# sylvainma/Summarizer

Hardware: NVIDIA B200
Metric: VASNet/DSN frames/sec fwd+bwd and knapsack-eval videos/sec at 1/2/4/8 B200 (higher is better)
Workload: dtype bf16 (tcgen05 operands, fp32 accumulate/softmax/LayerNorm); i32/u8 eval

## Files before the change

include/summarizer_b200.h:

```cpp
#ifndef SUMMARIZER_B200_H
#define SUMMARIZER_B200_H

#include <stdint.h>

#ifdef __cplusplus
extern "C" {
#endif

#define SMZ_OK 0
#define SMZ_ERR_ARG (-1)
#define SMZ_ERR_CUDA (-2)
#define SMZ_ERR_UNSUPPORTED (-3)
#define SMZ_ERR_NCCL (-4)
#define SMZ_ERR_DEVICE (-5)

#define SMZ_METHOD_KNAPSACK 0
#define SMZ_METHOD_RANK 1

#define SMZ_STATUS_VALUE_RANGE 1
#define SMZ_STATUS_INTERVALS 2
#define SMZ_STATUS_WEIGHT_RANGE 4

#define SMZ_FSCORE_CHUNK 2048

// ... 49 lines not shown

int smz_upsample(const smz_video_desc *desc, int n_videos, int max_n_frames, const float *scores,
                 const int32_t *picks, float *frame_scores, int32_t *status, void *stream);

#define SMZ_METRIC_SPEARMAN 0
#define SMZ_METRIC_KENDALL 1
typedef struct smz_corr_desc {
    int64_t m_off, u_off, u_ld, rank_off;
    int32_t n_frames, n_users, row0, reserved;
} smz_corr_desc;
int smz_rank_correlation(const smz_corr_desc *desc, int n_videos, int max_n_frames, int max_n_users,
                         const float *machine, const float *user, int metric, float *rank_ws, double *corr,
                         double *corr_avg, void *stream);

#define SMZ_OPTIM_MAX_TENSORS 64
typedef struct smz_optim_tensor {
    float *param, *grad, *exp_avg, *exp_avg_sq, *step;
    int64_t n;
} smz_optim_tensor;
int smz_grad_sqnorm_workspace_floats(const smz_optim_tensor *tensors, int n_tensors, int64_t *floats);
int smz_grad_sqnorm(const smz_optim_tensor *tensors, int n_tensors, float *sqnorm, float *ws, int64_t ws_floats, void *stream);
int smz_clip_grads(const smz_optim_tensor *tensors, int n_tensors, const float *sqnorm, float max_norm, void *stream);
int smz_adam_step(const smz_optim_tensor *tensors, int n_tensors, double lr, double beta1, double beta2, double eps,
                  double weight_decay, void *stream);
int smz_mse_loss(const float *scores, const float *target, int64_t n, float *loss, float *dscores, void *stream);

#define SMZ_GEMM_OUT_F32 1
#define SMZ_GEMM_RELU 2
#define SMZ_GEMM_RES_F32 4
#define SMZ_GEMM_BIAS_M 8
#define SMZ_GEMM_OUT_F16 2048
#define SMZ_GEMM_A_F16 4096
#define SMZ_GEMM_B_F16 8192
int smz_gemm_bf16_tn(const void *A, int64_t lda, const void *B, int64_t ldb, void *C, int64_t ldc, int M, int N,
                     int K, float alpha, const float *bias, const void *residual, int64_t ldr, int flags,
                     void *stream);
int smz_cvt_bf16_multi(const float *const *src, void *const *dst, const int64_t *n, int count, void *stream);
int smz_gemm_bf16(int a_mn, int b_mn, const void *A, int64_t lda, const void *B, int64_t ldb, void *C, int64_t ldc,
                  int M, int N, int K, float alpha, const float *bias, const void *residual, int64_t ldr, int flags,
                  void *stream);
int smz_gemm_bf16_split(int a_mn, int b_mn, const void *A, const void *A_lo, int64_t lda, const void *B,
                        const void *B_lo, int64_t ldb, void *C, void *C_lo, int64_t ldc, int M, int N, int K, float alpha,
                        const float *bias, const void *residual, int64_t ldr, int flags, void *stream);
int smz_split_bf16_multi(const float *const *src, void *const *hi, void *const *lo, const int64_t *n, int count,
                         void *stream);

#define SMZ_VASNET_STATUS_LOGIT_RANGE 1
#define SMZ_VASNET_STATUS_F16_RANGE 2
typedef struct smz_vasnet_params {
    const void *wqk, *wv, *wo, *w1;
    const float *b1, *w2, *b2, *ln_g, *ln_b;
    float scale, eps;
    int32_t aperture, ignore_self;
    const float *head_gw, *head_c;
    const void *w1g;
    const float *ln_c, *b1f;
    const void *wgv, *wgv16;
    int32_t *status;
    const void *wqk_lo, *wv_lo, *wo_lo, *w1_lo;
} smz_vasnet_params;
#define SMZ_VASNET_SPLIT 4

int smz_dropout_keep_masks(uint64_t *state, uint8_t *out, int64_t n, void *stream);
int smz_vasnet_workspace_bytes(const int32_t *h_cu_seqlens, int n_videos, int training, int x_is_bf16,
                               int64_t *bytes);
void smz_vasnet_set_exact_softmax(int on);
// ... 110 lines not shown
```

summarizer_b200/csrc/smz_gemm.cu:

```cuda
#include "smz_gemm.cuh"
#include "smz_tc.cuh"

#include <cudaTypedefs.h>
#include <stdlib.h>

namespace {

using namespace smztc;
using smz::GemmEpilogue;
using smz::GemmProblem;

constexpr int BM = 128;
constexpr int BN = smz::GEMM_BN, BK = smz::GEMM_BK;
constexpr int A_STAGE = BM * BK * 2;
constexpr int EPI_WARPS = 8;
constexpr int NUM_THREADS = 64 + 32 * EPI_WARPS;
constexpr int TMEM_COLS = 2 * BN;
constexpr int BAR_BYTES = 256;
constexpr int STG_BYTES = EPI_WARPS * 32 * 33 * 4;
static_assert(TMEM_COLS == 512, "TMEM allocation must be a power of two <= 512 columns");
template <bool PAIR> struct Cfg {
    static constexpr int STAGES = PAIR ? 5 : 3;
    static constexpr int B_ROWS = PAIR ? BN / 2 : BN;
    static constexpr int B_STAGE = B_ROWS * BK * 2;
    static constexpr int TILE_M = PAIR ? 2 * BM : BM;
    static constexpr int SMEM_BYTES = STAGES * (A_STAGE + B_STAGE) + BAR_BYTES + STG_BYTES + 1024;
};

struct Params {
    const GemmProblem *probs;
    GemmProblem single;
    int n_probs, total_tiles;
    GemmEpilogue epi;
};

struct Cursor {
    int p = -1;
    GemmProblem cur;
    __device__ __forceinline__ void seek(const Params &P, int tile) {
        if (P.probs == nullptr) { cur = P.single; return; }
        int q = p < 0 ? 0 : p;
        while (q + 1 < P.n_probs && tile >= __ldg(&P.probs[q + 1].tile0)) ++q;
        if (q != p) { p = q; cur = P.probs[q]; }
    }
};

__device__ __forceinline__ float4 ld_f4(const float *p) { return *reinterpret_cast<const float4 *>(p); }

enum { EPI_PLAIN = 0, EPI_HEAD = 1, EPI_EXP = 2, EPI_SPLIT = 3 };

template <bool A_MN, bool B_MN, bool PAIR, int EPI_T>
__global__ void __launch_bounds__(NUM_THREADS, 1)
gemm_kernel(const __grid_constant__ CUtensorMap tmA, const __grid_constant__ CUtensorMap tmB,
            const __grid_constant__ CUtensorMap tmA_lo, const __grid_constant__ CUtensorMap tmB_lo, const Params P) {
    constexpr bool SPLIT_OUT = EPI_T == EPI_SPLIT;
    constexpr int EPI = SPLIT_OUT ? (int)EPI_PLAIN : EPI_T;
    const int pass_a = P.epi.a_lo != 0 ? 1 : -1;
    const int pass_b = P.epi.b_lo != 0 ? (P.epi.a_lo != 0 ? 2 : 1) : -1;
    const int npass = 1 + (P.epi.a_lo != 0 ? 1 : 0) + (P.epi.b_lo != 0 ? 1 : 0);
    constexpr int STAGES = Cfg<PAIR>::STAGES, B_STAGE = Cfg<PAIR>::B_STAGE, B_ROWS = Cfg<PAIR>::B_ROWS;
    constexpr int TILE_M = Cfg<PAIR>::TILE_M;
    extern __shared__ uint8_t smem_raw[];
    uint8_t *smem = smem_raw + ((1024u - (smem_u32(smem_raw) & 1023u)) & 1023u);
    uint8_t *sA = smem;
    uint8_t *sB = smem + STAGES * A_STAGE;
    uint64_t *full = reinterpret_cast<uint64_t *>(smem + STAGES * (A_STAGE + B_STAGE));
    uint64_t *empty = full + STAGES;
    uint64_t *tfull = empty + STAGES;
    uint64_t *tempty = tfull + 2;
    uint32_t *tmem_slot = reinterpret_cast<uint32_t *>(tempty + 2);
    float *stg_all = reinterpret_cast<float *>(smem + STAGES * (A_STAGE + B_STAGE) + BAR_BYTES);

    smz::pdl_trigger();
    if (P.epi.gate != nullptr) {
        smz::pdl_wait();
        if (__ldg(P.epi.gate) == 0) return;
    }
    const int warp = __shfl_sync(0xffffffffu, threadIdx.x >> 5, 0), lane = threadIdx.x & 31;
    const int rank = PAIR ? (int)cluster_ctarank() : 0;
    const int first_tile = PAIR ? (int)(blockIdx.x >> 1) : (int)blockIdx.x;
    const int tile_step = PAIR ? (int)(gridDim.x >> 1) : (int)gridDim.x;
    if (PAIR) cluster_sync_all();
    if (warp == 0 && lane == 0) {
        tma_prefetch_desc(&tmA);
        tma_prefetch_desc(&tmB);
        if (npass > 1) { tma_prefetch_desc(&tmA_lo); tma_prefetch_desc(&tmB_lo); }
        for (int i = 0; i < STAGES; i++) { mbar_init(&full[i], PAIR ? 2 : 1); mbar_init(&empty[i], 1); }
        for (int i = 0; i < 2; i++) { mbar_init(&tfull[i], 1); mbar_init(&tempty[i], (PAIR ? 2 : 1) * 32 * EPI_WARPS); }
        fence_mbar_init();
    }
    if (warp == 1) { if (PAIR) tmem_alloc_pair<TMEM_COLS>(tmem_slot); else tmem_alloc<TMEM_COLS>(tmem_slot); }
    tc_fence_before();
    if (PAIR) cluster_sync_all(); else __syncthreads();
    tc_fence_after();
// ... 21 lines not shown
                        else if (rank == 0) mbar_arrive_expect_tx(&full[stage], 2 * (A_STAGE + B_STAGE));
                        else mbar_arrive_remote(&full[stage], 0);
                        if (A_MN) {
#pragma unroll
                            for (int j = 0; j < BM / 64; j++)
                                tma_load<PAIR>(sA + stage * A_STAGE + j * 8192, mapA, &full[stage], a_mn + 64 * j, a_k + kb * BK);
                        } else {
                            tma_load<PAIR>(sA + stage * A_STAGE, mapA, &full[stage], a_k + kb * BK, a_mn);
                        }
                        if (B_MN) {
#pragma unroll
                            for (int j = 0; j < B_ROWS / 64; j++)
                                tma_load<PAIR>(sB + stage * B_STAGE + j * 8192, mapB, &full[stage], b_mn + 64 * j, b_k + kb * BK);
                        } else {
                            tma_load<PAIR>(sB + stage * B_STAGE, mapB, &full[stage], b_k + kb * BK, b_mn);
                        }
                    }
                    __syncwarp();
                    if (++stage == STAGES) { stage = 0; phase ^= 1u; }
                }
            }
        }
    } else if (warp == 1) {
        if (rank == 0) {
            Cursor c;
            const uint32_t idesc = (make_idesc_bf16(TILE_M, BN) | (A_MN ? (1u << 15) : 0u) | (B_MN ? (1u << 16) : 0u))
                                   & ~(((P.epi.flags & smz::GEMM_A_F16) ? (1u << 7) : 0u) | ((P.epi.flags & smz::GEMM_B_F16) ? (1u << 10) : 0u));
            const uint32_t a_base = smem_u32(sA), b_base = smem_u32(sB);
            int stage = 0; uint32_t phase = 0;
            int it = 0;
            for (int tile = first_tile; tile < P.total_tiles; tile += tile_step, ++it) {
                c.seek(P, tile);
                const int nkb = ((c.cur.K + BK - 1) / BK) * npass;
                const int as = it & 1;
                mbar_wait(&tempty[as], (((uint32_t)it >> 1) & 1u) ^ 1u);
                tc_fence_after();
                const uint32_t d_tmem = tmem_base + (uint32_t)(as * BN);
                for (int kb = 0; kb < nkb; kb++) {
                    mbar_wait(&full[stage], phase);
                    tc_fence_after();
                    const uint32_t a_addr = a_base + stage * A_STAGE, b_addr = b_base + stage * B_STAGE;
                    const uint64_t adesc = A_MN ? make_mnmajor_sw128_desc(a_addr) : make_kmajor_sw128_desc(a_addr);
                    const uint64_t bdesc = B_MN ? make_mnmajor_sw128_desc(b_addr) : make_kmajor_sw128_desc(b_addr);
                    if (elect_one()) {
#pragma unroll
                        for (int k = 0; k < BK / 16; k++)
                            umma_bf16<PAIR>(d_tmem, adesc + (A_MN ? 128 : 2) * k, bdesc + (B_MN ? 128 : 2) * k, idesc,
                                            (uint32_t)((kb | k) != 0));
                        umma_commit<PAIR>(&empty[stage]);
                    }
                    __syncwarp();
                    if (++stage == STAGES) { stage = 0; phase ^= 1u; }
                }
                if (elect_one()) umma_commit<PAIR>(&tfull[as]);
                __syncwarp();
            }
        }
    } else {
        Cursor c;
        const int q = warp & 3;
        const int half = (warp - 2) >> 2;
        float *stg = stg_all + (warp - 2) * (32 * 33);
        const int row = q * 32 + lane;
        const float alpha = P.epi.alpha;
        const int flags = P.epi.flags;
        int it = 0;
        for (int tile = first_tile; tile < P.total_tiles; tile += tile_step, ++it) {
            c.seek(P, tile);
            const GemmProblem &g = c.cur;
            const int lt = tile - g.tile0;
            const int mt = lt / g.tiles_n, nt = lt - mt * g.tiles_n;
            const int as = it & 1;
            const int m = mt * TILE_M + rank * BM + row;
            const bool row_ok = m < g.M;
            const float bias_m = (P.epi.bias != nullptr && (flags & smz::GEMM_BIAS_M) && !(flags & (smz::GEMM_SCALE_M | smz::GEMM_SCALE_STATS)) && row_ok) ? __ldg(P.epi.bias + m) : 0.f;
            const bool out_f32 = flags & smz::GEMM_OUT_F32;
            const bool res_f32 = flags & smz::GEMM_RES_F32;
            const bool c_vec = ((g.c_off | (int64_t)g.ldc) & 7) == 0 && (reinterpret_cast<uintptr_t>(P.epi.C) & 15) == 0;
            const int64_t res_off = (flags & smz::GEMM_RES_AT_C) ? g.c_off : g.r_off;
            const int res_ld = (flags & smz::GEMM_RES_AT_C) ? g.ldc : g.ldr;
            const bool r_vec = ((res_off | (int64_t)res_ld) & 7) == 0 && (reinterpret_cast<uintptr_t>(P.epi.residual) & 15) == 0;
            const char *res_row = P.epi.residual == nullptr ? nullptr
                : reinterpret_cast<const char *>(P.epi.residual) + (res_off + (int64_t)m * res_ld) * (res_f32 ? 4 : 2);
            auto res_vec_ok = [&](int n0) { return res_row != nullptr && row_ok && r_vec && n0 + 32 <= g.N; };
            auto res_fetch = [&](int n0, uint4 (&buf)[8]) {
                if (!res_vec_ok(n0)) return;
                const uint4 *src = reinterpret_cast<const uint4 *>(res_row + (int64_t)n0 * (res_f32 ? 4 : 2));
#pragma unroll
                for (int j = 0; j < 8; j++)
                    if (res_f32 || j < 4) buf[j] = src[j];
            };
            uint4 rcur[8], rnext[8];
            float st1 = 0.f, st2 = 0.f, st3 = 0.f;
            constexpr bool do_exp = EPI == EPI_EXP;
            const int n_store = do_exp ? ((g.N + 63) & ~63) : g.N;
            float amax = 0.f;
            if (EPI == EPI_PLAIN && res_row != nullptr && row_ok) {
                const char *pf = res_row + (int64_t)(nt * BN + half * (BN / 2)) * (res_f32 ? 4 : 2);
                const int bytes = (BN / 2) * (res_f32 ? 4 : 2);
                for (int b = 0; b < bytes; b += 128)
                    asm volatile("prefetch.global.L2 [%0];" ::"l"(pf + b));
            }
            res_fetch(nt * BN + half * (BN / 2), rcur);
            float row_scale = 1.f, ln_mean = 0.f, ln_rstd = 1.f;
            if (EPI == EPI_PLAIN && row_ok && (flags & smz::GEMM_SCALE_M)) row_scale = __ldg(P.epi.bias + g.r_off + m);
            if (EPI == EPI_PLAIN && row_ok && (flags & smz::GEMM_SCALE_STATS)) {
                const int ns = P.epi.scale_slots > 0 ? P.epi.scale_slots : P.epi.stat_slots;
                const float *sp = P.epi.bias + (g.r_off + m) * ns * 3;
                float ssum = 0.f;
                for (int k = 0; k < ns; k++) ssum += __ldg(sp + 3 * k);
                row_scale = 1.f / ssum;
            }
            if (EPI == EPI_HEAD && row_ok && (flags & smz::GEMM_LN_FOLD)) {
                const float *sp = P.epi.ln_stats + (g.r_off + m) * P.epi.ln_slots * 3;
                float s1 = 0.f, s2 = 0.f;
                for (int k = 0; k < P.epi.ln_slots; k++) { s1 += __ldg(sp + 3 * k); s2 += __ldg(sp + 3 * k + 1); }
                const float inv_w = 1.f / (float)P.epi.ln_width;
                ln_mean = s1 * inv_w;
                ln_rstd = rsqrtf(fmaxf(s2 * inv_w - ln_mean * ln_mean, 0.f) + P.epi.ln_eps);
            }
            mbar_wait(&tfull[as], ((uint32_t)it >> 1) & 1u);
            tc_fence_after();
            for (int c0 = half * (BN / 2); c0 < (half + 1) * (BN / 2); c0 += 32) {
                const int n0 = nt * BN + c0;
                if (n0 >= n_store) break;
                uint32_t v[32];
                uint32_t lo_pk[SPLIT_OUT ? 16 : 1];
                __syncwarp();
                tmem_ld32(tmem_base + ((uint32_t)(q * 32) << 16) + (uint32_t)(as * BN + c0), v);
                if (c0 + 32 < (half + 1) * (BN / 2)) res_fetch(n0 + 32, rnext);
                tmem_ld_wait();
                if (row_ok) {
                float x[32];
#pragma unroll
                for (int j = 0; j < 32; j++) x[j] = alpha * __uint_as_float(v[j]);
                const bool full32 = n0 + 32 <= n_store;
                if constexpr (do_exp) {
                    const int ap = P.epi.aperture, ig = P.epi.ignore_self;
                    if (ap < 0 && !ig && n0 + 32 <= g.N) {
#pragma unroll
                        for (int j = 0; j < 32; j++) {
                            amax = fmaxf(amax, fabsf(x[j]));
                            x[j] = __expf(x[j]);
                        }
                    } else {
#pragma unroll
                        for (int j = 0; j < 32; j++) {
                            const int col = n0 + j;
                            float e = x[j];
                            bool live = col < g.N;
                            if (ig && col == m) live = false;
                            if (ap >= 0) {
                                int d = m - col; d = d < 0 ? -d : d;
                                if (d > ap || e * e == 0.f) live = false;
                            }
// ... 64 lines not shown
                }
                const bool f16 = EPI == EPI_PLAIN && (flags & smz::GEMM_OUT_F16) && n0 >= P.epi.f16_col0;
                if (f16 && !(flags & smz::GEMM_LN_STATS)) {
#pragma unroll
                    for (int j = 0; j < 32; j += 2) amax = fmaxf(amax, fmaxf(fabsf(x[j]), fabsf(x[j + 1])));
                }
                if (EPI == EPI_PLAIN && (flags & smz::GEMM_LN_STATS)) {
#pragma unroll
                    for (int j = 0; j < 32; j += 4) {
                        st1 += (x[j] + x[j + 1]) + (x[j + 2] + x[j + 3]);
                        st2 = fmaf(x[j], x[j], st2); st2 = fmaf(x[j + 1], x[j + 1], st2);
                        st2 = fmaf(x[j + 2], x[j + 2], st2); st2 = fmaf(x[j + 3], x[j + 3], st2);
                    }
                }
                if constexpr (EPI == EPI_HEAD) {
#pragma unroll
                    for (int j = 0; j < 32; j += 4) {
                        const float4 sw = ld_f4(P.epi.stat_w + n0 + j);
                        st1 += (x[j] + x[j + 1]) + (x[j + 2] + x[j + 3]);
                        st2 = fmaf(x[j], x[j], st2); st2 = fmaf(x[j + 1], x[j + 1], st2);
                        st2 = fmaf(x[j + 2], x[j + 2], st2); st2 = fmaf(x[j + 3], x[j + 3], st2);
                        st3 = fmaf(x[j], sw.x, st3); st3 = fmaf(x[j + 1], sw.y, st3);
                        st3 = fmaf(x[j + 2], sw.z, st3); st3 = fmaf(x[j + 3], sw.w, st3);
                    }
                }
                if constexpr (EPI == EPI_EXP) {
#pragma unroll
                    for (int j = 0; j < 32; j += 4) st1 += (x[j] + x[j + 1]) + (x[j + 2] + x[j + 3]);
                }
                if constexpr (EPI != EPI_HEAD) {
                const int64_t co = g.c_off + (int64_t)m * g.ldc + n0;
                if (out_f32) {
                    float *dst = reinterpret_cast<float *>(P.epi.C) + co;
                    if (full32) {
#pragma unroll
                        for (int j = 0; j < 32; j++) stg[lane * 33 + j] = x[j];
                    } else {
#pragma unroll
                        for (int j = 0; j < 32; j++) if (n0 + j < g.N) dst[j] = x[j];
                    }
                } else {
                    __nv_bfloat16 *dst = reinterpret_cast<__nv_bfloat16 *>(P.epi.C) + co;
                    if (full32 && c_vec) {
                        uint4 *pad = reinterpret_cast<uint4 *>(reinterpret_cast<uint32_t *>(stg) + lane * 20);
#pragma unroll
                        for (int j = 0; j < 32; j += 8)
                            pad[j >> 3] = f16 ?
                                make_uint4(pack_f16x2(x[j], x[j + 1]), pack_f16x2(x[j + 2], x[j + 3]),
                                           pack_f16x2(x[j + 4], x[j + 5]), pack_f16x2(x[j + 6], x[j + 7])) :
                                make_uint4(pack_bf16x2(x[j], x[j + 1]), pack_bf16x2(x[j + 2], x[j + 3]),
                                           pack_bf16x2(x[j + 4], x[j + 5]), pack_bf16x2(x[j + 6], x[j + 7]));
                        if constexpr (SPLIT_OUT) {
#pragma unroll
                            for (int j = 0; j < 32; j += 2) {
                                const uint32_t hi = pack_bf16x2(x[j], x[j + 1]);
                                lo_pk[j >> 1] = pack_bf16x2(x[j] - __uint_as_float(hi << 16), x[j + 1] - __uint_as_float(hi & 0xffff0000u));
                            }
                        }
                    } else if (f16) {
#pragma unroll
                        for (int j = 0; j < 32; j++) if (n0 + j < g.N) reinterpret_cast<__half *>(dst)[j] = __float2half_rn(x[j]);
                    } else {
#pragma unroll
                        for (int j = 0; j < 32; j++) if (n0 + j < g.N) {
                            const __nv_bfloat16 hi = __float2bfloat16_rn(x[j]);
                            dst[j] = hi;
                            if (SPLIT_OUT) dst[P.epi.c_lo + j] = __float2bfloat16_rn(x[j] - __bfloat162float(hi));
                        }
                    }
                }
                }
                }
                if (EPI == EPI_PLAIN && out_f32 && n0 + 32 <= g.N) {
                    __syncwarp();
                    const int m_base = m - lane;
                    float *base = reinterpret_cast<float *>(P.epi.C) + g.c_off + n0 + lane;
#pragma unroll 8
                    for (int r = 0; r < 32; r++)
                        if (m_base + r < g.M) base[(int64_t)(m_base + r) * g.ldc] = stg[r * 33 + lane];
                    __syncwarp();
                }
                if (EPI != EPI_HEAD && !out_f32 && n0 + 32 <= n_store && c_vec) {
                    __syncwarp();
                    const int m_base = m - lane;
                    const int sub = lane >> 2, part = lane & 3;
                    __nv_bfloat16 *base = reinterpret_cast<__nv_bfloat16 *>(P.epi.C) + g.c_off + n0 + part * 8;
#pragma unroll
                    for (int i = 0; i < 4; i++) {
                        const int r = 8 * i + sub;
                        const uint4 w4 = *reinterpret_cast<const uint4 *>(reinterpret_cast<const uint32_t *>(stg) + r * 20 + part * 4);
                        if (m_base + r < g.M) *reinterpret_cast<uint4 *>(base + (int64_t)(m_base + r) * g.ldc) = w4;
                    }
                    __syncwarp();
                    if constexpr (SPLIT_OUT) {
                        if (row_ok) {
                            uint4 *pad = reinterpret_cast<uint4 *>(reinterpret_cast<uint32_t *>(stg) + lane * 20);
#pragma unroll
                            for (int j = 0; j < 4; j++) pad[j] = make_uint4(lo_pk[4 * j], lo_pk[4 * j + 1], lo_pk[4 * j + 2], lo_pk[4 * j + 3]);
                        }
                        __syncwarp();
#pragma unroll
                        for (int i = 0; i < 4; i++) {
                            const int r = 8 * i + sub;
                            const uint4 w4 = *reinterpret_cast<const uint4 *>(reinterpret_cast<const uint32_t *>(stg) + r * 20 + part * 4);
                            if (m_base + r < g.M) *reinterpret_cast<uint4 *>(base + P.epi.c_lo + (int64_t)(m_base + r) * g.ldc) = w4;
                        }
                        __syncwarp();
                    }
                }
#pragma unroll
                for (int j = 0; j < 8; j++) rcur[j] = rnext[j];
            }
            if ((EPI != EPI_PLAIN || (flags & smz::GEMM_LN_STATS)) && row_ok) {
                const int slots = P.epi.stat_slots > 0 ? P.epi.stat_slots : 2 * g.tiles_n;
                float *so = P.epi.stat_out + ((g.r_off + m) * slots + (nt * 2 + half)) * 3;
                so[0] = st1; so[1] = st2; so[2] = st3;
            }
            if (do_exp && P.epi.guard != nullptr && !(amax <= 80.f)) atomicOr(P.epi.guard, P.epi.guard_bit);
            if (EPI == EPI_PLAIN && (flags & smz::GEMM_OUT_F16) && P.epi.guard != nullptr && row_ok &&
                !(((flags & smz::GEMM_LN_STATS) ? st2 : amax * amax) <= 3.6e9f))
                atomicOr(P.epi.guard, P.epi.guard_bit);
            tc_fence_before();
            if (PAIR) mbar_arrive_remote(&tempty[as], 0); else mbar_arrive(&tempty[as]);
        }
    }
    __syncwarp();
    tc_fence_before();
    if (PAIR) cluster_sync_all(); else __syncthreads();
    if (warp == 1) {
        tc_fence_after();
        if (PAIR) tmem_dealloc_pair<TMEM_COLS>(tmem_base); else tmem_dealloc<TMEM_COLS>(tmem_base);
    }
}

PFN_cuTensorMapEncodeTiled_v12000 encode_fn() {
    static PFN_cuTensorMapEncodeTiled_v12000 fn = nullptr;
    if (fn == nullptr) {
        void *p = nullptr;
        cudaDriverEntryPointQueryResult q;
        if (cudaGetDriverEntryPoint("cuTensorMapEncodeTiled", &p, cudaEnableDefault, &q) == cudaSuccess &&
            q == cudaDriverEntryPointSuccess)
            fn = reinterpret_cast<PFN_cuTensorMapEncodeTiled_v12000>(p);
    }
    return fn;
}

int make_map(CUtensorMap *m, const void *base, int64_t rows, int64_t cols, int64_t ld, int box_rows) {
    PFN_cuTensorMapEncodeTiled_v12000 enc = encode_fn();
    if (enc == nullptr) return smz::fail(SMZ_ERR_CUDA, "cuTensorMapEncodeTiled is not available from the driver");
    if ((reinterpret_cast<uintptr_t>(base) & 15) != 0 || (ld & 7) != 0 || rows <= 0 || cols <= 0)
        return smz::fail(SMZ_ERR_ARG, "gemm operand must be 16-byte aligned with a leading dimension multiple of 8 "
                         "(base %p, ld %lld, %lld x %lld)", base, (long long)ld, (long long)rows, (long long)cols);
    const cuuint64_t dims[2] = {(cuuint64_t)cols, (cuuint64_t)rows};
    const cuuint64_t strides[1] = {(cuuint64_t)ld * 2};
// ... 1 lines not shown
    const cuuint32_t estr[2] = {1, 1};
    const CUresult r = enc(m, CU_TENSOR_MAP_DATA_TYPE_BFLOAT16, 2, const_cast<void *>(base), dims, strides, box, estr,
                           CU_TENSOR_MAP_INTERLEAVE_NONE, CU_TENSOR_MAP_SWIZZLE_128B, CU_TENSOR_MAP_L2_PROMOTION_L2_256B,
                           CU_TENSOR_MAP_FLOAT_OOB_FILL_NONE);
    if (r != CUDA_SUCCESS) return smz::fail(SMZ_ERR_CUDA, "cuTensorMapEncodeTiled failed (%d)", (int)r);
    return SMZ_OK;
}

}

namespace smz {

int make_bf16_map(CUtensorMap *m, const void *base, int64_t rows, int64_t cols, int64_t ld, int box_rows) {
    return make_map(m, base, rows, cols, ld, box_rows);
}

int gemm_bf16_tn(const void *A, int64_t a_rows, int64_t a_cols, int64_t lda, const void *B, int64_t b_rows,
                 int64_t b_cols, int64_t ldb, const GemmProblem *d_probs, int n_probs, int total_tiles,
                 const GemmProblem &single, const GemmEpilogue &epi, cudaStream_t st) {
    return gemm_bf16(false, false, A, a_rows, a_cols, lda, B, b_rows, b_cols, ldb, d_probs, n_probs, total_tiles, single,
                     epi, st);
}

bool gemm_pair_mode() {
    static int v = -1;
    if (v < 0) { const char *e = getenv("SMZ_GEMM_PAIR"); v = (e != nullptr && e[0] == '0') ? 0 : 1; }
    return v == 1;
}

int gemm_tile_m() { return gemm_pair_mode() ? 2 * BM : BM; }

int gemm_tiles(int M, int N) { return ((M + gemm_tile_m() - 1) / gemm_tile_m()) * ((N + GEMM_BN - 1) / GEMM_BN); }

template <bool PAIR>
static int launch_variant(bool a_mn, bool b_mn, const CUtensorMap &ma, const CUtensorMap &mb, const CUtensorMap &ma_lo,
                          const CUtensorMap &mb_lo, const Params &P, int total_tiles, cudaStream_t st) {
    typedef void (*kern_t)(const CUtensorMap, const CUtensorMap, const CUtensorMap, const CUtensorMap, const Params);
    const int f = P.epi.flags;
    const int epi = (f & GEMM_EXP) ? EPI_EXP : (f & GEMM_ROWSTATS) ? EPI_HEAD
                    : (P.epi.c_lo != 0 && !(f & GEMM_OUT_F32)) ? EPI_SPLIT : EPI_PLAIN;
    kern_t kern;
    if (epi == EPI_SPLIT) {
        if (f & (GEMM_OUT_F16 | GEMM_LN_STATS)) return fail(SMZ_ERR_UNSUPPORTED, "gemm: hi + lo output planes are bf16, without row statistics");
        if ((P.epi.c_lo & 7) != 0) return fail(SMZ_ERR_ARG, "gemm: c_lo must be a multiple of 8 elements");
        kern = a_mn ? (b_mn ? (kern_t)gemm_kernel<true, true, PAIR, EPI_SPLIT> : (kern_t)gemm_kernel<true, false, PAIR, EPI_SPLIT>)
                    : (b_mn ? (kern_t)gemm_kernel<false, true, PAIR, EPI_SPLIT> : (kern_t)gemm_kernel<false, false, PAIR, EPI_SPLIT>);
    } else if (epi != EPI_PLAIN) {
        if (a_mn || b_mn) return fail(SMZ_ERR_UNSUPPORTED, "gemm: the fused head / exp epilogues exist for K-major operands only");
        if (epi == EPI_HEAD && (!(f & GEMM_NO_STORE) || P.epi.stat_w == nullptr || P.epi.stat_out == nullptr))
            return fail(SMZ_ERR_ARG, "gemm: GEMM_ROWSTATS needs GEMM_NO_STORE, stat_w and stat_out");
        if (epi == EPI_EXP && (!(f & GEMM_ROWSTATS) || (f & GEMM_OUT_F32) || P.epi.stat_out == nullptr))
            return fail(SMZ_ERR_ARG, "gemm: GEMM_EXP writes bf16 and needs GEMM_ROWSTATS + stat_out");
        kern = epi == EPI_HEAD ? (kern_t)gemm_kernel<false, false, PAIR, EPI_HEAD> : (kern_t)gemm_kernel<false, false, PAIR, EPI_EXP>;
    } else {
        kern = a_mn ? (b_mn ? (kern_t)gemm_kernel<true, true, PAIR, EPI_PLAIN> : (kern_t)gemm_kernel<true, false, PAIR, EPI_PLAIN>)
                    : (b_mn ? (kern_t)gemm_kernel<false, true, PAIR, EPI_PLAIN> : (kern_t)gemm_kernel<false, false, PAIR, EPI_PLAIN>);
    }
    const int variant = epi == EPI_SPLIT ? 6 + (a_mn ? 2 : 0) + (b_mn ? 1 : 0) : epi != EPI_PLAIN ? 3 + epi : (a_mn ? 2 : 0) + (b_mn ? 1 : 0);
    static bool attr_set[64][10] = {{false}};
    int dev = 0;
    SMZ_CUDA_CHECK(cudaGetDevice(&dev));
    if (dev >= 0 && dev < 64 && !attr_set[dev][variant]) {
        SMZ_CUDA_CHECK(cudaFuncSetAttribute((const void *)kern, cudaFuncAttributeMaxDynamicSharedMemorySize, Cfg<PAIR>::SMEM_BYTES));
        attr_set[dev][variant] = true;
    }
    const int sms = sm_count();
    cudaLaunchConfig_t cfg = {};
    cfg.blockDim = dim3(NUM_THREADS);
    cfg.dynamicSmemBytes = Cfg<PAIR>::SMEM_BYTES;
    cfg.stream = st;
    cudaLaunchAttribute attr[2];
    int n_attr = 0;
    if (PAIR) {
        const int pairs = total_tiles < sms / 2 ? total_tiles : sms / 2;
        cfg.gridDim = dim3(2 * pairs);
        attr[n_attr].id = cudaLaunchAttributeClusterDimension;
        attr[n_attr].val.clusterDim.x = 2; attr[n_attr].val.clusterDim.y = 1; attr[n_attr].val.clusterDim.z = 1;
        ++n_attr;
    } else {
        cfg.gridDim = dim3(total_tiles < sms ? total_tiles : sms);
    }
    if (pdl_enabled() && total_tiles < (PAIR ? sms / 2 : sms)) {
        attr[n_attr].id = cudaLaunchAttributeProgrammaticStreamSerialization;
        attr[n_attr].val.programmaticStreamSerializationAllowed = 1;
        ++n_attr;
    }
    cfg.attrs = attr; cfg.numAttrs = n_attr;
    SMZ_CUDA_CHECK(cudaLaunchKernelEx(&cfg, kern, ma, mb, ma_lo, mb_lo, P));
    return SMZ_OK;
}

int gemm_bf16(bool a_mn, bool b_mn, const void *A, int64_t a_rows, int64_t a_cols, int64_t lda, const void *B,
              int64_t b_rows, int64_t b_cols, int64_t ldb, const GemmProblem *d_probs, int n_probs, int total_tiles,
              const GemmProblem &single, const GemmEpilogue &epi, cudaStream_t st) {
    if (total_tiles <= 0) return SMZ_OK;
    SMZ_REQUIRE(A && B && epi.C, "gemm: NULL operand");
    SMZ_REQUIRE(d_probs != nullptr || n_probs == 1, "gemm: a batch needs a device problem array");
    alignas(64) CUtensorMap ma, mb;
    const bool pair = gemm_pair_mode();
    int rc = make_map(&ma, A, a_rows, a_cols, lda, a_mn ? 64 : BM);
    if (rc != SMZ_OK) return rc;
    rc = make_map(&mb, B, b_rows, b_cols, ldb, b_mn ? 64 : (pair ? BN / 2 : BN));
// ... 80 lines not shown
```

summarizer_b200/csrc/smz_gemm.cuh:

```cuda
#pragma once
#include <cuda.h>

#include "smz_common.cuh"

namespace smz {

struct GemmProblem {
    int32_t a_row0, a_col0, b_row0, b_col0;
    int32_t M, N, K;
    int32_t tile0;
    int64_t c_off;
    int64_t r_off;
    int32_t ldc, ldr;
    int32_t tiles_n;
    int32_t pad;
};
static_assert(sizeof(GemmProblem) == 64, "GemmProblem layout");

enum : int {
    GEMM_OUT_F32 = 1,
    GEMM_RELU = 2,
    GEMM_RES_F32 = 4,
    GEMM_BIAS_M = 8,
    GEMM_ROWSTATS = 16,
    GEMM_NO_STORE = 32,
    GEMM_EXP = 64,
    GEMM_SCALE_M = 128,
    GEMM_SCALE_STATS = 256,
    GEMM_LN_STATS = 512,
    GEMM_OUT_F16 = 2048,
    GEMM_A_F16 = 4096,
    GEMM_B_F16 = 8192,
    GEMM_RES_AT_C = 16384,
    GEMM_LN_FOLD = 1024,
};

struct GemmEpilogue {
    void *C;
    const float *bias;
    const void *residual;
    float alpha;
    int flags;
    const float *stat_w = nullptr;
    float *stat_out = nullptr;
    int stat_slots = 0;
    int scale_slots = 0;
    int aperture = -1, ignore_self = 0;
    int *guard = nullptr;
    int guard_bit = 1;
    int f16_col0 = 0;
    const int *gate = nullptr;
    const float *ln_stats = nullptr;
    const float *ln_c = nullptr;
    int ln_slots = 0, ln_width = 0;
    float ln_eps = 0.f;
    int64_t a_lo = 0, b_lo = 0, c_lo = 0;
};

constexpr int GEMM_BN = 256;
constexpr int GEMM_BK = 64;

int gemm_tile_m();
int gemm_tiles(int M, int N);

int gemm_bf16_tn(const void *A, int64_t a_rows, int64_t a_cols, int64_t lda, const void *B, int64_t b_rows,
                 int64_t b_cols, int64_t ldb, const GemmProblem *d_probs, int n_probs, int total_tiles,
// ... 10 lines not shown
```

summarizer_b200/csrc/smz_vasnet.cu:

```cuda
#include <stdlib.h>

#include <map>
#include <mutex>
#include <utility>
#include <vector>

#include "smz_gemm.cuh"
#include "smz_rows.cuh"

namespace {

using smz::GemmEpilogue;
using smz::GemmProblem;
using smz::kFeat;
typedef __nv_bfloat16 bf16;

constexpr int kRowChunk = 32768;
int64_t logit_budget() {
    static int64_t v = -1;
    if (v < 0) { const char *e = getenv("SMZ_VASNET_LOGIT_MELEMS"); v = (e != nullptr && atoi(e) > 0) ? ((int64_t)atoi(e) << 20) : (68ll << 20); }
    return v;
}

inline int64_t up(int64_t x, int64_t m) { return (x + m - 1) / m * m; }
// ... 133 lines not shown

struct SideStreams { cudaStream_t s[2]; cudaEvent_t fork, join[2], ev[6]; bool ok; };
SideStreams *side_streams(cudaStream_t caller) {
    static std::mutex mu;
    static std::map<std::pair<int, cudaStream_t>, SideStreams *> table;
    int dev = 0;
    if (cudaGetDevice(&dev) != cudaSuccess) return nullptr;
    std::lock_guard<std::mutex> lock(mu);
    SideStreams *&slot = table[std::make_pair(dev, caller)];
    if (slot == nullptr) {
        SideStreams *t = new SideStreams();
        for (int i = 0; i < 2; i++) {
            if (cudaStreamCreateWithFlags(&t->s[i], cudaStreamNonBlocking) != cudaSuccess) return nullptr;
            if (cudaEventCreateWithFlags(&t->join[i], cudaEventDisableTiming) != cudaSuccess) return nullptr;
        }
        if (cudaEventCreateWithFlags(&t->fork, cudaEventDisableTiming) != cudaSuccess) return nullptr;
        for (int i = 0; i < 6; i++)
            if (cudaEventCreateWithFlags(&t->ev[i], cudaEventDisableTiming) != cudaSuccess) return nullptr;
        t->ok = true;
        slot = t;
    }
    return slot;
}

GemmProblem dense_problem(int M, int N, int K, int ldc, int ldr) {
    GemmProblem g = {};
    g.M = M; g.N = N; g.K = K; g.ldc = ldc; g.ldr = ldr;
    g.tiles_n = (N + smz::GEMM_BN - 1) / smz::GEMM_BN;
    return g;
}

int fast_chunk(const Plan &pl, const Chunk &c, const int32_t *cu, const smz_vasnet_params *p, const void *xb, const void *res,
               bool x_bf16, bf16 *gv, bf16 *P, bf16 *y16, float *sstat, float *lnstat, float *hstat, const GemmProblem *d_probs,
               float *scores, cudaStream_t st) {
    const int R = c.rows, n = pl.n_videos;
    const int f16 = x_bf16 ? 0 : (smz::GEMM_A_F16 | smz::GEMM_B_F16);
    int rc;
    smz::profile_mark(st, "gemm_proj");
    {
        GemmEpilogue e{gv, nullptr, nullptr, 1.f, f16 | (x_bf16 ? 0 : smz::GEMM_OUT_F16)};
        e.f16_col0 = kFeat; e.guard = p->status; e.guard_bit = SMZ_VASNET_STATUS_F16_RANGE;
        rc = smz::gemm_bf16_tn(xb, R, kFeat, kFeat, x_bf16 ? p->wgv : p->wgv16, 2 * kFeat, kFeat, kFeat, nullptr, 1,
                               smz::gemm_tiles(R, 2 * kFeat), dense_problem(R, 2 * kFeat, kFeat, 2 * kFeat, 0), e, st);
        if (rc != SMZ_OK) return rc;
        SMZ_DEBUG_STEP(st, "gemm_proj");
    }
    int slots = 0;
    for (const Sub &s : c.subs) { const int k = 2 * ((s.ld + 255) / 256); if (k > slots) slots = k; }
    bool ragged = false;
    for (int v = c.v0; v < c.v1; v++) ragged |= 2 * ((cu[v + 1] - cu[v] + 255) / 256) != slots;
    if (ragged) SMZ_CUDA_CHECK(cudaMemsetAsync(sstat, 0, (int64_t)R * slots * 3 * 4, st));
    constexpr int kLnSlots = 2 * kFeat / smz::GEMM_BN;
    for (const Sub &s : c.subs) {
        const int nv = s.v1 - s.v0;
        int tiles_s = 0, tiles_pv = 0;
        for (int v = s.v0; v < s.v1; v++) {
            const int T = cu[v + 1] - cu[v];
            tiles_s += smz::gemm_tiles(T, T);
            tiles_pv += smz::gemm_tiles(T, kFeat);
        }
        smz::profile_mark(st, "gemm_logits");
        {
            GemmEpilogue e{P, nullptr, nullptr, p->scale, smz::GEMM_EXP | smz::GEMM_ROWSTATS | f16};
            e.stat_out = sstat; e.stat_slots = slots; e.aperture = p->aperture; e.ignore_self = p->ignore_self;
            e.guard = p->status; e.guard_bit = SMZ_VASNET_STATUS_LOGIT_RANGE;
            rc = smz::gemm_bf16_tn(gv, R, 2 * kFeat, 2 * kFeat, xb, R, kFeat, kFeat, d_probs + s.v0, nv, tiles_s, GemmProblem{}, e, st);
            if (rc != SMZ_OK) return rc;
            SMZ_DEBUG_STEP(st, "gemm_logits_exp");
        }
        smz::profile_mark(st, "gemm_pv");
        {
            GemmEpilogue e{y16, sstat, res, 1.f, smz::GEMM_SCALE_STATS | smz::GEMM_RES_AT_C | (x_bf16 ? 0 : smz::GEMM_RES_F32) |
                                                 smz::GEMM_LN_STATS | smz::GEMM_OUT_F16};
            e.scale_slots = slots; e.stat_out = lnstat; e.stat_slots = kLnSlots;
            e.guard = p->status; e.guard_bit = SMZ_VASNET_STATUS_F16_RANGE;
            rc = smz::gemm_bf16(false, true, P, s.rows, s.ld, s.ld, gv, R, 2 * kFeat, 2 * kFeat, d_probs + n + s.v0, nv, tiles_pv,
                                GemmProblem{}, e, st);
            if (rc != SMZ_OK) return rc;
            SMZ_DEBUG_STEP(st, "gemm_pv");
        }
    }
    smz::profile_mark(st, "gemm_k1");
    {
        GemmEpilogue e{hstat, p->b1f, nullptr, 1.f, smz::GEMM_RELU | smz::GEMM_OUT_F32 | smz::GEMM_ROWSTATS | smz::GEMM_NO_STORE |
                                                   smz::GEMM_LN_FOLD | smz::GEMM_A_F16 | smz::GEMM_B_F16};
        e.stat_w = p->head_gw; e.stat_out = hstat;
        e.ln_stats = lnstat; e.ln_c = p->ln_c; e.ln_slots = kLnSlots; e.ln_width = kFeat; e.ln_eps = p->eps;
        rc = smz::gemm_bf16_tn(y16, R, kFeat, kFeat, p->w1g, kFeat, kFeat, kFeat, nullptr, 1, smz::gemm_tiles(R, kFeat),
                               dense_problem(R, kFeat, kFeat, kFeat, 0), e, st);
        if (rc != SMZ_OK) return rc;
        SMZ_DEBUG_STEP(st, "gemm_k1");
    }
    smz::profile_mark(st, "head");
    rc = smz::launch_head_from_stats(hstat, kLnSlots, p->head_c, p->eps, R, scores, st);
    if (rc != SMZ_OK) return rc;
    SMZ_DEBUG_STEP(st, "head");
    smz::profile_mark(st, "");
    return SMZ_OK;
}

}

namespace { int g_exact_softmax = 0; }
extern "C" void smz_vasnet_set_exact_softmax(int on) { g_exact_softmax = on; }

extern "C" int smz_vasnet_workspace_bytes(const int32_t *h_cu_seqlens, int n_videos, int training, int x_is_bf16,
                                          int64_t *bytes) {
    SMZ_REQUIRE(bytes != nullptr, "bytes is NULL");
    Plan pl;
    SMZ_REQUIRE(!(training & SMZ_VASNET_SPLIT) || (training & 1), "vasnet: the split-bf16 mode uses the training layout (training = 1 | SMZ_VASNET_SPLIT)");
    int rc = make_plan(h_cu_seqlens, n_videos, (training & ~SMZ_VASNET_SPLIT) != 0, x_is_bf16 != 0, &pl);
    if (rc != SMZ_OK) return rc;
    *bytes = (training & SMZ_VASNET_SPLIT) ? 2 * pl.total : pl.total;
    return SMZ_OK;
}

extern "C" int smz_vasnet_launch_count(const int32_t *h_cu_seqlens, int n_videos, int training, int x_is_bf16,
                                       int64_t *launches) {
// ... 77 lines not shown
    }
    int chunk_index = 0;
    for (const Chunk &c : pl.chunks) {
        const int R = c.rows;
        const int64_t Rpad = up(R, 8);
        const int64_t rb = training ? c.row0 : 0;
        const int lane_id = ss != nullptr ? (chunk_index & 1) : 0;
        ++chunk_index;
        if (ss != nullptr) st = ss->s[lane_id];
        const int64_t lb = (int64_t)lane_id * pl.lane_bytes;
        auto lane = [&](auto *ptr) { return reinterpret_cast<decltype(ptr)>(reinterpret_cast<uint8_t *>(ptr) + lb); };
        const int qld = training ? 2 * kFeat : 3 * kFeat;
        qk = lane(qk0) + rb * 2 * kFeat; vt = lane(vt0) + c.vt_off; o = lane(o0) + rb * kFeat; y = lane(y0) + rb * kFeat;
        yn = lane(yn0) + rb * kFeat; h = lane(h0) + rb * kFeat; S = lane(S0) + c.lg_off; P = lane(P0) + c.lg_off;
        alpha = lane(alpha0) + c.lg_off;
        stats = training ? stats0 + rb : nullptr;
        const bf16 *xb;
        if (x_is_bf16) {
            xb = reinterpret_cast<const bf16 *>(x) + (int64_t)c.row0 * kFeat;
        } else {
            bf16 *dst = reinterpret_cast<bf16 *>(w + pl.off_xb + lb) + rb * kFeat;
            const float *src = reinterpret_cast<const float *>(x) + (int64_t)c.row0 * kFeat;
            rc = fast ? smz::launch_cvt_f16(src, dst, (int64_t)R * kFeat, p->status, SMZ_VASNET_STATUS_F16_RANGE, st)
                      : smz::launch_cvt_bf16(src, dst, (int64_t)R * kFeat, st, XLO);
            if (rc != SMZ_OK) return rc;
        SMZ_DEBUG_STEP(st, "cvt");
            xb = dst;
        }
        if (fast) {
            const void *res = x_is_bf16 ? (const void *)(reinterpret_cast<const bf16 *>(x) + (int64_t)c.row0 * kFeat)
                                        : (const void *)(reinterpret_cast<const float *>(x) + (int64_t)c.row0 * kFeat);
            rc = fast_chunk(pl, c, h_cu_seqlens, p, xb, res, x_is_bf16 != 0, qk, P, yn, reinterpret_cast<float *>(w + pl.off_sstat + lb),
                            reinterpret_cast<float *>(w + pl.off_lnstat + lb), reinterpret_cast<float *>(w + pl.off_hstat + lb),
                            d_probs, scores + c.row0, st);
            if (rc != SMZ_OK) return rc;
            continue;
        }
        SideStreams *fs = (training && !smz::profile_enabled() && !smz::debug_sync_enabled()) ? side_streams(caller) : nullptr;
        cudaStream_t st_v = st;
        if (fs != nullptr) {
            SMZ_CUDA_CHECK(cudaEventRecord(fs->ev[0], st));
            SMZ_CUDA_CHECK(cudaStreamWaitEvent(fs->s[0], fs->ev[0], 0));
            st_v = fs->s[0];
        }
        smz::profile_mark(st, "gemm_qk");
        const bool wqkv_packed = reinterpret_cast<const bf16 *>(p->wv) == reinterpret_cast<const bf16 *>(p->wqk) + 2 * kFeat * kFeat;
        if (!training && wqkv_packed) {
            rc = smz::gemm_bf16_tn(xb, R, kFeat, kFeat, p->wqk, 3 * kFeat, kFeat, kFeat, nullptr, 1, smz::gemm_tiles(R, 3 * kFeat),
                                   dense_problem(R, 3 * kFeat, kFeat, 3 * kFeat, 0), GemmEpilogue{qk, nullptr, nullptr, 1.f, 0}, st);
            if (rc != SMZ_OK) return rc;
            SMZ_DEBUG_STEP(st, "gemm_qkv");
        } else {
            rc = smz::gemm_bf16_tn(xb, R, kFeat, kFeat, p->wqk, 2 * kFeat, kFeat, kFeat, nullptr, 1, smz::gemm_tiles(R, 2 * kFeat),
                                   dense_problem(R, 2 * kFeat, kFeat, qld, 0),
                                   split(GemmEpilogue{qk, nullptr, nullptr, 1.f, 0}, XLO, wlo(p->wqk_lo, p->wqk), LO), st);
            if (rc != SMZ_OK) return rc;
            SMZ_DEBUG_STEP(st, "gemm_qk");
            smz::profile_mark(st, "gemm_vt");
            if (training)
                rc = smz::gemm_bf16_tn(p->wv, kFeat, kFeat, kFeat, xb, R, kFeat, kFeat, nullptr, 1, smz::gemm_tiles(kFeat, R),
                                       dense_problem(kFeat, R, kFeat, (int)Rpad, 0),
                                       split(GemmEpilogue{vt, nullptr, nullptr, 1.f, 0}, wlo(p->wv_lo, p->wv), XLO, LO), st_v);
            else
                rc = smz::gemm_bf16_tn(xb, R, kFeat, kFeat, p->wv, kFeat, kFeat, kFeat, nullptr, 1, smz::gemm_tiles(R, kFeat),
                                       dense_problem(R, kFeat, kFeat, qld, 0), GemmEpilogue{qk + 2 * kFeat, nullptr, nullptr, 1.f, 0}, st_v);
            if (rc != SMZ_OK) return rc;
            if (fs != nullptr) SMZ_CUDA_CHECK(cudaEventRecord(fs->ev[1], st_v));
// ... 242 lines not shown
```

Baseline: 37600.

## Add co-resident two-CTA-per-SM variant of the CTA-pair GEMM for fast path

Adds a second configuration of the CTA-pair tcgen05 GEMM kernel, requested through a new CORESIDENT flag. It uses 4 epilogue warps that each process both column halves, a single TMEM accumulator of 256 columns, and 3 pipeline stages, so two CTAs fit on one SM. A host-side check of shared memory and register occupancy only selects it when two blocks really fit per SM. The VASNet fast-chunk GEMMs set the flag when a two-lane side-stream context is present, so concurrent chunks can share SMs. In exchange each CTA loses the double-buffered accumulator overlap and the staged, coalesced fp32 store path, and it has fewer epilogue warps.

```diff
diff --git a/include/summarizer_b200.h b/include/summarizer_b200.h
--- a/include/summarizer_b200.h
+++ b/include/summarizer_b200.h
@@ -105,6 +105,7 @@
 #define SMZ_GEMM_OUT_F16 2048
 #define SMZ_GEMM_A_F16 4096
 #define SMZ_GEMM_B_F16 8192
+#define SMZ_GEMM_CORESIDENT 32768
 int smz_gemm_bf16_tn(const void *A, int64_t lda, const void *B, int64_t ldb, void *C, int64_t ldc, int M, int N,
                      int K, float alpha, const float *bias, const void *residual, int64_t ldr, int flags,
                      void *stream);
diff --git a/summarizer_b200/csrc/smz_gemm.cu b/summarizer_b200/csrc/smz_gemm.cu
--- a/summarizer_b200/csrc/smz_gemm.cu
+++ b/summarizer_b200/csrc/smz_gemm.cu
@@ -13,18 +13,24 @@
 constexpr int BM = 128;
 constexpr int BN = smz::GEMM_BN, BK = smz::GEMM_BK;
 constexpr int A_STAGE = BM * BK * 2;
-constexpr int EPI_WARPS = 8;
-constexpr int NUM_THREADS = 64 + 32 * EPI_WARPS;
-constexpr int TMEM_COLS = 2 * BN;
 constexpr int BAR_BYTES = 256;
-constexpr int STG_BYTES = EPI_WARPS * 32 * 33 * 4;
-static_assert(TMEM_COLS == 512, "TMEM allocation must be a power of two <= 512 columns");
-template <bool PAIR> struct Cfg {
-    static constexpr int STAGES = PAIR ? 5 : 3;
+constexpr int PAD16_WORDS = 32 * 20;
+template <bool PAIR, bool CORES = false> struct Cfg {
+    static_assert(PAIR || !CORES, "the co-resident form is a CTA-pair kernel");
+    static constexpr int STAGES = CORES ? 3 : PAIR ? 5 : 3;
     static constexpr int B_ROWS = PAIR ? BN / 2 : BN;
     static constexpr int B_STAGE = B_ROWS * BK * 2;
     static constexpr int TILE_M = PAIR ? 2 * BM : BM;
-    static constexpr int SMEM_BYTES = STAGES * (A_STAGE + B_STAGE) + BAR_BYTES + STG_BYTES + 1024;
+    static constexpr int EPI_WARPS = CORES ? 4 : 8;
+    static constexpr int HALVES = CORES ? 2 : 1;
+    static constexpr int NUM_THREADS = 64 + 32 * EPI_WARPS;
+    static constexpr int MIN_BLOCKS = CORES ? 2 : 1;
+    static constexpr int ACCS = CORES ? 1 : 2;
+    static constexpr int TMEM_COLS = ACCS * BN;
+    static constexpr int STG_WORDS = CORES ? PAD16_WORDS : 32 * 33;
+    static constexpr int SMEM_BYTES = STAGES * (A_STAGE + B_STAGE) + BAR_BYTES + EPI_WARPS * STG_WORDS * 4 + 1024;
+    static_assert(TMEM_COLS == 256 || TMEM_COLS == 512, "TMEM allocation must be a power of two <= 512 columns");
+    static_assert(!CORES || 2 * (SMEM_BYTES + 1024) <= 228 * 1024, "two co-resident CTAs must fit one SM's shared memory");
 };
 
 struct Params {
@@ -49,8 +55,8 @@
 
 enum { EPI_PLAIN = 0, EPI_HEAD = 1, EPI_EXP = 2, EPI_SPLIT = 3 };
 
-template <bool A_MN, bool B_MN, bool PAIR, int EPI_T>
-__global__ void __launch_bounds__(NUM_THREADS, 1)
+template <bool A_MN, bool B_MN, bool PAIR, int EPI_T, bool CORES = false>
+__global__ void __launch_bounds__(Cfg<PAIR, CORES>::NUM_THREADS, Cfg<PAIR, CORES>::MIN_BLOCKS)
 gemm_kernel(const __grid_constant__ CUtensorMap tmA, const __grid_constant__ CUtensorMap tmB,
             const __grid_constant__ CUtensorMap tmA_lo, const __grid_constant__ CUtensorMap tmB_lo, const Params P) {
     constexpr bool SPLIT_OUT = EPI_T == EPI_SPLIT;
@@ -58,8 +64,9 @@
     const int pass_a = P.epi.a_lo != 0 ? 1 : -1;
     const int pass_b = P.epi.b_lo != 0 ? (P.epi.a_lo != 0 ? 2 : 1) : -1;
     const int npass = 1 + (P.epi.a_lo != 0 ? 1 : 0) + (P.epi.b_lo != 0 ? 1 : 0);
-    constexpr int STAGES = Cfg<PAIR>::STAGES, B_STAGE = Cfg<PAIR>::B_STAGE, B_ROWS = Cfg<PAIR>::B_ROWS;
-    constexpr int TILE_M = Cfg<PAIR>::TILE_M;
+    using Cf = Cfg<PAIR, CORES>;
+    constexpr int STAGES = Cf::STAGES, B_STAGE = Cf::B_STAGE, B_ROWS = Cf::B_ROWS;
+    constexpr int TILE_M = Cf::TILE_M, EPI_WARPS = Cf::EPI_WARPS, ACCS = Cf::ACCS, TMEM_COLS = Cf::TMEM_COLS;
     extern __shared__ uint8_t smem_raw[];
     uint8_t *smem = smem_raw + ((1024u - (smem_u32(smem_raw) & 1023u)) & 1023u);
     uint8_t *sA = smem;
@@ -147,8 +154,8 @@
             for (int tile = first_tile; tile < P.total_tiles; tile += tile_step, ++it) {
                 c.seek(P, tile);
                 const int nkb = ((c.cur.K + BK - 1) / BK) * npass;
-                const int as = it & 1;
-                mbar_wait(&tempty[as], (((uint32_t)it >> 1) & 1u) ^ 1u);
+                const int as = it % ACCS;
+                mbar_wait(&tempty[as], (((uint32_t)(it / ACCS)) & 1u) ^ 1u);
                 tc_fence_after();
                 const uint32_t d_tmem = tmem_base + (uint32_t)(as * BN);
                 for (int kb = 0; kb < nkb; kb++) {
@@ -174,8 +181,8 @@
     } else {
         Cursor c;
         const int q = warp & 3;
-        const int half = (warp - 2) >> 2;
-        float *stg = stg_all + (warp - 2) * (32 * 33);
+        const int half0 = CORES ? 0 : (warp - 2) >> 2;
+        float *stg = stg_all + (warp - 2) * Cf::STG_WORDS;
         const int row = q * 32 + lane;
         const float alpha = P.epi.alpha;
         const int flags = P.epi.flags;
@@ -185,7 +192,7 @@
             const GemmProblem &g = c.cur;
             const int lt = tile - g.tile0;
             const int mt = lt / g.tiles_n, nt = lt - mt * g.tiles_n;
-            const int as = it & 1;
+            const int as = it % ACCS;
             const int m = mt * TILE_M + rank * BM + row;
             const bool row_ok = m < g.M;
             const float bias_m = (P.epi.bias != nullptr && (flags & smz::GEMM_BIAS_M) && !(flags & (smz::GEMM_SCALE_M | smz::GEMM_SCALE_STATS)) && row_ok) ? __ldg(P.epi.bias + m) : 0.f;
@@ -206,17 +213,15 @@
                     if (res_f32 || j < 4) buf[j] = src[j];
             };
             uint4 rcur[8], rnext[8];
-            float st1 = 0.f, st2 = 0.f, st3 = 0.f;
             constexpr bool do_exp = EPI == EPI_EXP;
             const int n_store = do_exp ? ((g.N + 63) & ~63) : g.N;
-            float amax = 0.f;
             if (EPI == EPI_PLAIN && res_row != nullptr && row_ok) {
-                const char *pf = res_row + (int64_t)(nt * BN + half * (BN / 2)) * (res_f32 ? 4 : 2);
-                const int bytes = (BN / 2) * (res_f32 ? 4 : 2);
+                const char *pf = res_row + (int64_t)(nt * BN + half0 * (BN / 2)) * (res_f32 ? 4 : 2);
+                const int bytes = Cf::HALVES * (BN / 2) * (res_f32 ? 4 : 2);
                 for (int b = 0; b < bytes; b += 128)
                     asm volatile("prefetch.global.L2 [%0];" ::"l"(pf + b));
             }
-            res_fetch(nt * BN + half * (BN / 2), rcur);
+            res_fetch(nt * BN + half0 * (BN / 2), rcur);
             float row_scale = 1.f, ln_mean = 0.f, ln_rstd = 1.f;
             if (EPI == EPI_PLAIN && row_ok && (flags & smz::GEMM_SCALE_M)) row_scale = __ldg(P.epi.bias + g.r_off + m);
             if (EPI == EPI_PLAIN && row_ok && (flags & smz::GEMM_SCALE_STATS)) {
@@ -234,8 +239,12 @@
                 ln_mean = s1 * inv_w;
                 ln_rstd = rsqrtf(fmaxf(s2 * inv_w - ln_mean * ln_mean, 0.f) + P.epi.ln_eps);
             }
-            mbar_wait(&tfull[as], ((uint32_t)it >> 1) & 1u);
+            mbar_wait(&tfull[as], ((uint32_t)(it / ACCS)) & 1u);
             tc_fence_after();
+            for (int half = half0; half < half0 + Cf::HALVES; half++) {
+            if (half != half0) res_fetch(nt * BN + half * (BN / 2), rcur);
+            float st1 = 0.f, st2 = 0.f, st3 = 0.f;
+            float amax = 0.f;
             for (int c0 = half * (BN / 2); c0 < (half + 1) * (BN / 2); c0 += 32) {
                 const int n0 = nt * BN + c0;
                 if (n0 >= n_store) break;
@@ -366,7 +375,7 @@
                 const int64_t co = g.c_off + (int64_t)m * g.ldc + n0;
                 if (out_f32) {
                     float *dst = reinterpret_cast<float *>(P.epi.C) + co;
-                    if (full32) {
+                    if (!CORES && full32) {
 #pragma unroll
                         for (int j = 0; j < 32; j++) stg[lane * 33 + j] = x[j];
                     } else {
@@ -405,7 +414,7 @@
                 }
                 }
                 }
-                if (EPI == EPI_PLAIN && out_f32 && n0 + 32 <= g.N) {
+                if (!CORES && EPI == EPI_PLAIN && out_f32 && n0 + 32 <= g.N) {
                     __syncwarp();
                     const int m_base = m - lane;
                     float *base = reinterpret_cast<float *>(P.epi.C) + g.c_off + n0 + lane;
@@ -454,6 +463,7 @@
             if (EPI == EPI_PLAIN && (flags & smz::GEMM_OUT_F16) && P.epi.guard != nullptr && row_ok &&
                 !(((flags & smz::GEMM_LN_STATS) ? st2 : amax * amax) <= 3.6e9f))
                 atomicOr(P.epi.guard, P.epi.guard_bit);
+            }
             tc_fence_before();
             if (PAIR) mbar_arrive_remote(&tempty[as], 0); else mbar_arrive(&tempty[as]);
         }
@@ -521,10 +531,31 @@
 
 int gemm_tiles(int M, int N) { return ((M + gemm_tile_m() - 1) / gemm_tile_m()) * ((N + GEMM_BN - 1) / GEMM_BN); }
 
+bool gemm_coresident_enabled() {
+    static int v = -1;
+    if (v < 0) { const char *e = getenv("SMZ_GEMM_CORESIDENT"); v = (e != nullptr && e[0] == '0') ? 0 : 1; }
+    return v == 1;
+}
+
+typedef void (*kern_t)(const CUtensorMap, const CUtensorMap, const CUtensorMap, const CUtensorMap, const Params);
+
+static bool two_per_sm(kern_t kern, int threads, int smem_bytes) {
+    int dev = 0, smem_sm = 0, reserved = 0, regs_sm = 0;
+    cudaFuncAttributes fa;
+    if (cudaGetDevice(&dev) != cudaSuccess || cudaFuncGetAttributes(&fa, (const void *)kern) != cudaSuccess ||
+        cudaDeviceGetAttribute(&smem_sm, cudaDevAttrMaxSharedMemoryPerMultiprocessor, dev) != cudaSuccess ||
+        cudaDeviceGetAttribute(&reserved, cudaDevAttrReservedSharedMemoryPerBlock, dev) != cudaSuccess ||
+        cudaDeviceGetAttribute(&regs_sm, cudaDevAttrMaxRegistersPerMultiprocessor, dev) != cudaSuccess) {
+        (void)cudaGetLastError();
+        return false;
+    }
+    const int regs_cta = threads / 32 * ((fa.numRegs * 32 + 255) / 256 * 256);
+    return 2 * (smem_bytes + (int)fa.sharedSizeBytes + reserved) <= smem_sm && 2 * regs_cta <= regs_sm;
+}
+
 template <bool PAIR>
 static int launch_variant(bool a_mn, bool b_mn, const CUtensorMap &ma, const CUtensorMap &mb, const CUtensorMap &ma_lo,
                           const CUtensorMap &mb_lo, const Params &P, int total_tiles, cudaStream_t st) {
-    typedef void (*kern_t)(const CUtensorMap, const CUtensorMap, const CUtensorMap, const CUtensorMap, const Params);
     const int f = P.epi.flags;
     const int epi = (f & GEMM_EXP) ? EPI_EXP : (f & GEMM_ROWSTATS) ? EPI_HEAD
                     : (P.epi.c_lo != 0 && !(f & GEMM_OUT_F32)) ? EPI_SPLIT : EPI_PLAIN;
@@ -553,10 +584,29 @@
         SMZ_CUDA_CHECK(cudaFuncSetAttribute((const void *)kern, cudaFuncAttributeMaxDynamicSharedMemorySize, Cfg<PAIR>::SMEM_BYTES));
         attr_set[dev][variant] = true;
     }
+    int threads = Cfg<PAIR>::NUM_THREADS, smem_bytes = Cfg<PAIR>::SMEM_BYTES;
+    if constexpr (PAIR) {
+        if ((f & GEMM_CORESIDENT) && gemm_coresident_enabled() && !a_mn && epi != EPI_SPLIT && dev >= 0 && dev < 64) {
+            using CC = Cfg<true, true>;
+            const int cv = epi == EPI_PLAIN ? (b_mn ? 1 : 0) : 1 + epi;
+            const kern_t ck = epi == EPI_HEAD ? (kern_t)gemm_kernel<false, false, true, EPI_HEAD, true>
+                              : epi == EPI_EXP ? (kern_t)gemm_kernel<false, false, true, EPI_EXP, true>
+                              : b_mn ? (kern_t)gemm_kernel<false, true, true, EPI_PLAIN, true>
+                                     : (kern_t)gemm_kernel<false, false, true, EPI_PLAIN, true>;
+            static signed char fits[64][4] = {{0}};
+            if (fits[dev][cv] == 0) {
+                SMZ_CUDA_CHECK(cudaFuncSetAttribute((const void *)ck, cudaFuncAttributeMaxDynamicSharedMemorySize, CC::SMEM_BYTES));
+                SMZ_CUDA_CHECK(cudaFuncSetAttribute((const void *)ck, cudaFuncAttributePreferredSharedMemoryCarveout,
+                                                    (int)cudaSharedmemCarveoutMaxShared));
+                fits[dev][cv] = two_per_sm(ck, CC::NUM_THREADS, CC::SMEM_BYTES) ? 1 : -1;
+            }
+            if (fits[dev][cv] > 0) { kern = ck; threads = CC::NUM_THREADS; smem_bytes = CC::SMEM_BYTES; }
+        }
+    }
     const int sms = sm_count();
     cudaLaunchConfig_t cfg = {};
-    cfg.blockDim = dim3(NUM_THREADS);
-    cfg.dynamicSmemBytes = Cfg<PAIR>::SMEM_BYTES;
+    cfg.blockDim = dim3(threads);
+    cfg.dynamicSmemBytes = smem_bytes;
     cfg.stream = st;
     cudaLaunchAttribute attr[2];
     int n_attr = 0;
diff --git a/summarizer_b200/csrc/smz_gemm.cuh b/summarizer_b200/csrc/smz_gemm.cuh
--- a/summarizer_b200/csrc/smz_gemm.cuh
+++ b/summarizer_b200/csrc/smz_gemm.cuh
@@ -32,6 +32,7 @@
     GEMM_A_F16 = 4096,
     GEMM_B_F16 = 8192,
     GEMM_RES_AT_C = 16384,
+    GEMM_CORESIDENT = 32768,
     GEMM_LN_FOLD = 1024,
 };
 
diff --git a/summarizer_b200/csrc/smz_vasnet.cu b/summarizer_b200/csrc/smz_vasnet.cu
--- a/summarizer_b200/csrc/smz_vasnet.cu
+++ b/summarizer_b200/csrc/smz_vasnet.cu
@@ -189,13 +189,14 @@
 
 int fast_chunk(const Plan &pl, const Chunk &c, const int32_t *cu, const smz_vasnet_params *p, const void *xb, const void *res,
                bool x_bf16, bf16 *gv, bf16 *P, bf16 *y16, float *sstat, float *lnstat, float *hstat, const GemmProblem *d_probs,
-               float *scores, cudaStream_t st) {
+               float *scores, bool two_lanes, cudaStream_t st) {
     const int R = c.rows, n = pl.n_videos;
     const int f16 = x_bf16 ? 0 : (smz::GEMM_A_F16 | smz::GEMM_B_F16);
+    const int cores = two_lanes ? smz::GEMM_CORESIDENT : 0;
     int rc;
     smz::profile_mark(st, "gemm_proj");
     {
-        GemmEpilogue e{gv, nullptr, nullptr, 1.f, f16 | (x_bf16 ? 0 : smz::GEMM_OUT_F16)};
+        GemmEpilogue e{gv, nullptr, nullptr, 1.f, f16 | cores | (x_bf16 ? 0 : smz::GEMM_OUT_F16)};
         e.f16_col0 = kFeat; e.guard = p->status; e.guard_bit = SMZ_VASNET_STATUS_F16_RANGE;
         rc = smz::gemm_bf16_tn(xb, R, kFeat, kFeat, x_bf16 ? p->wgv : p->wgv16, 2 * kFeat, kFeat, kFeat, nullptr, 1,
                                smz::gemm_tiles(R, 2 * kFeat), dense_problem(R, 2 * kFeat, kFeat, 2 * kFeat, 0), e, st);
@@ -218,7 +219,7 @@
         }
         smz::profile_mark(st, "gemm_logits");
         {
-            GemmEpilogue e{P, nullptr, nullptr, p->scale, smz::GEMM_EXP | smz::GEMM_ROWSTATS | f16};
+            GemmEpilogue e{P, nullptr, nullptr, p->scale, smz::GEMM_EXP | smz::GEMM_ROWSTATS | f16 | cores};
             e.stat_out = sstat; e.stat_slots = slots; e.aperture = p->aperture; e.ignore_self = p->ignore_self;
             e.guard = p->status; e.guard_bit = SMZ_VASNET_STATUS_LOGIT_RANGE;
             rc = smz::gemm_bf16_tn(gv, R, 2 * kFeat, 2 * kFeat, xb, R, kFeat, kFeat, d_probs + s.v0, nv, tiles_s, GemmProblem{}, e, st);
@@ -228,7 +229,7 @@
         smz::profile_mark(st, "gemm_pv");
         {
             GemmEpilogue e{y16, sstat, res, 1.f, smz::GEMM_SCALE_STATS | smz::GEMM_RES_AT_C | (x_bf16 ? 0 : smz::GEMM_RES_F32) |
-                                                 smz::GEMM_LN_STATS | smz::GEMM_OUT_F16};
+                                                 smz::GEMM_LN_STATS | smz::GEMM_OUT_F16 | cores};
             e.scale_slots = slots; e.stat_out = lnstat; e.stat_slots = kLnSlots;
             e.guard = p->status; e.guard_bit = SMZ_VASNET_STATUS_F16_RANGE;
             rc = smz::gemm_bf16(false, true, P, s.rows, s.ld, s.ld, gv, R, 2 * kFeat, 2 * kFeat, d_probs + n + s.v0, nv, tiles_pv,
@@ -240,7 +241,7 @@
     smz::profile_mark(st, "gemm_k1");
     {
         GemmEpilogue e{hstat, p->b1f, nullptr, 1.f, smz::GEMM_RELU | smz::GEMM_OUT_F32 | smz::GEMM_ROWSTATS | smz::GEMM_NO_STORE |
-                                                   smz::GEMM_LN_FOLD | smz::GEMM_A_F16 | smz::GEMM_B_F16};
+                                                   smz::GEMM_LN_FOLD | smz::GEMM_A_F16 | smz::GEMM_B_F16 | cores};
         e.stat_w = p->head_gw; e.stat_out = hstat;
         e.ln_stats = lnstat; e.ln_c = p->ln_c; e.ln_slots = kLnSlots; e.ln_width = kFeat; e.ln_eps = p->eps;
         rc = smz::gemm_bf16_tn(y16, R, kFeat, kFeat, p->w1g, kFeat, kFeat, kFeat, nullptr, 1, smz::gemm_tiles(R, kFeat),
@@ -384,7 +385,7 @@
                                         : (const void *)(reinterpret_cast<const float *>(x) + (int64_t)c.row0 * kFeat);
             rc = fast_chunk(pl, c, h_cu_seqlens, p, xb, res, x_is_bf16 != 0, qk, P, yn, reinterpret_cast<float *>(w + pl.off_sstat + lb),
                             reinterpret_cast<float *>(w + pl.off_lnstat + lb), reinterpret_cast<float *>(w + pl.off_hstat + lb),
-                            d_probs, scores + c.row0, st);
+                            d_probs, scores + c.row0, ss != nullptr, st);
             if (rc != SMZ_OK) return rc;
             continue;
         }
```

New measurement: 32310 (median of 6 runs). 14.1% lower.
